# Fahien/rayca

Hardware: AMD Instinct MI355X
Metric: Mrays/sec (primary+shadow), 1920x1080 Sponza 1spp (higher is better)
Workload: dtype f32; 1 GPU; sponza-STAND-IN procedural atrium 271,568 tris, 1920x1080, primary + 1 shadow ray (Pathtracer max_depth=1, NEE, 1 point light), 1 spp; width=1920, height=1080, triangles=271568, bvh_nodes=135379, bvh_built_on=gpu (bvh_build.hip; same tree as the host builder), rays_per_frame=4146938, frames_in_flight=4, tiling=rows in bands of 8 dealt over 1 rank(s), frame_gather=none, launched_by=single process

## Files before the change

### rayca_amd/csrc/kernels.hip

```cpp
#include "no_pk.hpp"
RAYCA_NO_PK_BEGIN
#include <hip/hip_runtime.h>
#include "device_types.hpp"
RAYCA_NO_PK_END

namespace rayca {
namespace {

RAYCA_NO_PK_BEGIN
#include "trace_core.inc"

template <int MODE, bool GEN0, bool ORDERED, bool FUSED, bool FAST, bool SPH, bool WIDE, bool SPILL, bool STATS, bool HALF>
__global__ __launch_bounds__(kBlock, MODE == kModeFlat ? RAYCA_MIN_WAVES_FLAT : RAYCA_MIN_WAVES) void k_generation(DevScene sc, FrameParams fp, uint32_t* heads, const QueuedRay* in_rays,
                                                       const uint32_t* in_count, QueuedRay* out_rays, uint32_t* out_count,
                                                       PathBuffers pb, uint32_t depth, uint8_t* rgba8, float4* rgba32f,
                                                       TraceCounters* counters, TraceLaunch tl) {
  extern __shared__ uint32_t lds_stack[];
  NodeStack<SPILL> stack = make_stack<SPILL>(lds_stack, tl, rc_bid() * kBlock + rc_tid());
  float4* const ctx_slot = reinterpret_cast<float4*>(lds_stack + tl.lds_entries * kBlock) + rc_tid();
  constexpr bool PARK = RAYCA_PARK_CTX && MODE == kModePath;
  const uint32_t lane = __lane_id();
  const uint32_t home = xcc_id();
  WorkCursor wc{};
  const uint32_t total = GEN0 ? fp.tile_count : (*in_count + 63u) / 64u;
  LaneCounters cnt{};
  uint32_t n_shaded = 0, n_shadow = 0, n_bounce = 0;
  const bool collect_emissive = GEN0 ? true : (fp.direct_sampler == RAYCA_SAMPLER_NONE);
  const uint32_t nee_lights = (MODE == kModePath && fp.direct_sampler == RAYCA_SAMPLER_NEE) ? sc.light_count : 0u;

  for (;;) {
    const uint32_t batch = next_batch(heads, total, home, wc, tl.ticket);
    if (batch == RAYCA_NONE) break;
    bool live;
    uint32_t p = 0, key = 0;
    DRay ray;
    if (GEN0) {
      const uint32_t ty = batch / fp.tiles_x, tx = batch - ty * fp.tiles_x;
      const uint32_t x = tx * kTileW + (lane & (kTileW - 1u)), r = ty * kTileH + (lane >> RAYCA_TILE_W_LOG2);
      live = x < fp.width && r < fp.rows;
      const uint32_t y = ((r / fp.band) * fp.parts + fp.part) * fp.band + (r % fp.band);
      p = r * fp.width + x;
      if (live) {
        ray = camera_ray(fp, x, y);
        key = rng_root(fp.seed, y * fp.width + x, fp.sample);
      }
    } else {
      const uint32_t i = batch * 64u + lane;
      live = i < *in_count;
      if (live) {
        const QueuedRay q = in_rays[i];
        ray = make_ray(point3(q.ox, q.oy, q.oz), vec3(q.dx, q.dy, q.dz));
        p = q.pixel;
        key = q.key;
      }
    }
    const size_t slot = (size_t)depth * pb.npix + p;
    bool in_shadow = false;
    float t_stop = FLT_MAX;
    ShadeCtx cx;
    Color ns_x = black();
    Color direct = black();
    uint32_t li = 0, k = 0, dim = 0;
    const bool has_pixel = live;
    bool tail = false;

    while (live) {
      DHit hit;
      constexpr int kLeaveK = !ORDERED ? 0 : (MODE == kModeFlat ? RAYCA_LEAVE_K_CAMERA : (GEN0 ? RAYCA_LEAVE_K_PATH0 : RAYCA_LEAVE_K_BOUNCE));
      constexpr int kSlackForm = MODE == kModeFlat ? kSlackAlways : (GEN0 ? kSlackPerWave : kSlackNever);
      const bool found = trace<ORDERED, FAST, SPH, WIDE, SPILL, STATS, HALF, kLeaveK, kSlackForm>(sc, ray, t_stop, stack, hit, cnt);
      if (!in_shadow) {
        if (!found) {
          if (FUSED) direct = black() + black();
          else pb.state[slot] = kVertexNone;
          live = false;
        } else {
          n_shaded++;
          Color color;
          bool emissive;
          shade_hit<SPH>(sc, ray, hit, MODE == kModePath, color, emissive, cx);
          if (MODE == kModeFlat) {
            if (FUSED) direct = black() + color;
            else {
              pb.direct[slot] = as_f4(color);
              pb.state[slot] = kVertexEmissive;
            }
            live = false;
          } else if (collect_emissive && emissive) {
            pb.direct[slot] = as_f4(color);
            pb.state[slot] = kVertexEmissive;
            live = false;
          } else {
            in_shadow = true;
            if (PARK) {
              park_ctx(ctx_slot, cx);
              ctx_slot[6 * kBlock] = as_f4(black());
            }
          }
        }
      } else {
        bool lit;
        if (t_stop == FLT_MAX) {
          lit = false;
          if (found) {
            const uint32_t hm = sc.ext[hit.prim].material;
            lit = hm != RAYCA_NONE && hm < sc.material_count && sc.materials[hm].emissive != 0u;
          }
        } else {
          lit = !(found && hit.t < t_stop);
        }
        if (PARK) {
          const Color sum = as_color(ctx_slot[6 * kBlock]) + (lit ? as_color(ctx_slot[5 * kBlock]) : black());
          ctx_slot[6 * kBlock] = as_f4(sum);
        } else {
          direct = direct + (lit ? ns_x : black());
        }
        if (++k == fp.light_samples) {
          k = 0;
          ++li;
        }
      }
      if (live && in_shadow) {
        bool pending = false;
        while (li < nee_lights) {
          if (PARK) cx = unpark_ctx(ctx_slot);
          const NeeSample ns = nee_prepare(sc, fp, cx, li, k, key, dim, ray);
          const bool irrelevant = ORDERED && nee_irrelevant(ns);
          if (STATS) {
            const unsigned long long m = __ballot(irrelevant);
            if (m != 0ull && lane == (uint32_t)__ffsll((long long)m) - 1u) atomicAdd(&counters->nee_irrelevant, (unsigned long long)__popcll(m));
          }
          if (irrelevant && fp.nee_skip) {
            if (++k == fp.light_samples) {
              k = 0;
              ++li;
            }
            continue;
          }
          if (PARK) ctx_slot[5 * kBlock] = as_f4(ns.x);
          else ns_x = ns.x;
          t_stop = ns.t_stop;
          pending = true;
          break;
        }
        if (!pending) {
          tail = true;
          live = false;
        }
      }
    }
    if (FUSED) {
      if (has_pixel) finalize_pixel(fp, direct, p, rgba8, rgba32f);
    } else if (MODE == kModePath) {
      bool want_bounce = false;
      QueuedRay next{};
      if (tail) {
        const uint32_t limit = fp.direct_sampler != RAYCA_SAMPLER_NONE ? fp.max_depth - 1u : fp.max_depth;
        const bool hemi = fp.indirect_sampler == RAYCA_SAMPLER_HEMISPHERE;
        F4 sdir = vec3(0.0f, 0.0f, 0.0f);
        if (depth < limit) {
          const float e1 = rng_f32(key, dim++), e2 = rng_f32(key, dim++);
          const float theta = hemi ? rc_acosf(e1) : rc_acosf(sqrtf(e1));
          const float omega_a = 2.0f * kPi * e2;
          const float st = rc_sinf(theta);
          sdir = vec3(rc_cosf(omega_a) * st, rc_sinf(omega_a) * st, rc_cosf(theta));
        }
        if (PARK) {
          cx = unpark_ctx(ctx_slot);
          direct = as_color(ctx_slot[6 * kBlock]);
        }
        pb.direct[slot] = as_f4(direct);
        if (depth < limit) {
          const F4 w = cx.normal;
          const F4 a = close(w, vec3(0, 1, 0)) ? vec3(1, 0, 0) : vec3(0, 1, 0);
          const F4 u = normalized(cross(a, w));
          F4 v = cross(w, u);
          if (hemi) v = normalized(v);
          const F4 omega_i = (sdir.x * u + sdir.y * v) + sdir.z * w;
          const Color brdf = surf_brdf(cx, omega_i);
          Color factor;
          if (hemi) factor = ((2.0f * kPi) * brdf) * clampf(dot(cx.normal, omega_i), 0.0f, 1.0f);
          else factor = kPi * brdf;
          pb.brdf[slot] = as_f4(factor);
          pb.state[slot] = kVertexLit;
          if (depth + 1u < fp.max_depth) {
            want_bounce = true;
            next.ox = cx.next_origin.x; next.oy = cx.next_origin.y; next.oz = cx.next_origin.z;
            next.dx = omega_i.x; next.dy = omega_i.y; next.dz = omega_i.z;
            next.pixel = p;
            next.key = rng_child(key, 0u);
          }
        } else {
          pb.state[slot] = kVertexLitNoIndirect;
        }
      }
      n_shadow += (uint32_t)__popcll(__ballot(tail)) * nee_lights * fp.light_samples;
      n_bounce += (uint32_t)__popcll(__ballot(want_bounce));
      push_ray(want_bounce, next, out_rays, out_count);
    }
  }
  if (STATS) {
    unsigned long long b = cnt.boxes, t = cnt.tris, sh = n_shaded, sb = cnt.slot_boxes, stt = cnt.slot_tris;
    for (int off = 32; off > 0; off >>= 1) {
      b += __shfl_down(b, off);
      t += __shfl_down(t, off);
      sh += __shfl_down(sh, off);
      sb += __shfl_down(sb, off);
      stt += __shfl_down(stt, off);
    }
    if (lane == 0) {
      atomicAdd(&counters->boxes, b);
      atomicAdd(&counters->tris, t);
      atomicAdd(&counters->shaded, sh);
      atomicAdd(&counters->box_slots, sb);
      atomicAdd(&counters->tri_slots, stt);
    }
  }
  if (MODE == kModePath) {
    const unsigned long long s2 = n_shadow, b2 = n_bounce;
    if (lane == 0 && (s2 | b2)) {
      atomicAdd(&counters->shadow, s2);
      atomicAdd(&counters->bounce, b2);
    }
  }
}

__global__ __launch_bounds__(kBlock) void k_resolve(FrameParams fp, PathBuffers pb, uint32_t depths, float4* accum, uint8_t* rgba8, float4* rgba32f,
                                                    uint32_t* clear, uint32_t clear_words) {
  if (clear && rc_bid() == 0)
    for (uint32_t i = rc_tid(); i < clear_words; i += rc_bdim()) clear[i] = 0u;
  const uint32_t p = rc_bid() * rc_bdim() + rc_tid();
  if (p >= pb.npix) return;
  bool some = false;
  Color L = black();
  for (int g = (int)depths - 1; g >= 0; --g) {
    const size_t slot = (size_t)g * pb.npix + p;
    const uint32_t st = pb.state[slot];
    if (st == kVertexNone) {
      some = false;
    } else if (st == kVertexEmissive) {
      some = true;
      L = as_color(pb.direct[slot]);
    } else {
      const Color direct = as_color(pb.direct[slot]);
      Color indirect = black();
      if (st == kVertexLit) {
        Color li = black();
        if (some) {
          const Color factor = as_color(pb.brdf[slot]);
          const Color x = (factor * L) * 1.0f;
          li = li + x;
        }
        indirect = indirect + li / (float)fp.light_samples;
      }
      L = direct + indirect;
      some = true;
    }
  }
  const Color c = some ? L : black();
  const Color prev = fp.sample == 0 ? black() : as_color(accum[p]);
  const Color acc = prev + c;
  if (fp.sample + 1u == fp.spp) finalize_pixel(fp, acc, p, rgba8, rgba32f);
  else accum[p] = as_f4(acc);
}

template <bool ORDERED, bool FAST, bool SPH, bool WIDE, bool SPILL, bool STATS>
__global__ __launch_bounds__(kBlock, RAYCA_TRACE_MIN_WAVES) void k_trace_rays(DevScene sc, const float* rays, uint32_t count, float* t_out, uint32_t* prim_out, float* uv_out,
                                                       TraceCounters* counters, TraceLaunch tl) {
  extern __shared__ uint32_t lds_stack[];
  NodeStack<SPILL> stack = make_stack<SPILL>(lds_stack, tl, rc_bid() * kBlock + rc_tid());
  const uint32_t i = rc_bid() * rc_bdim() + rc_tid();
  LaneCounters cnt{};
  if (i < count) {
    const float* r = rays + 6ull * i;
    const DRay ray = make_ray(point3(r[0], r[1], r[2]), vec3(r[3], r[4], r[5]));
    DHit hit;
    const bool found = trace<ORDERED, FAST, SPH, WIDE, SPILL, STATS, false, 0, kSlackAlways>(sc, ray, FLT_MAX, stack, hit, cnt);
    t_out[i] = found ? hit.t : FLT_MAX;
    prim_out[i] = found ? hit.prim : RAYCA_NONE;
    uv_out[2 * i] = found ? hit.u : 0.0f;
    uv_out[2 * i + 1] = found ? hit.v : 0.0f;
  }
  if (STATS) {
    unsigned long long b = cnt.boxes, t = cnt.tris;
    for (int off = 32; off > 0; off >>= 1) {
      b += __shfl_down(b, off);
      t += __shfl_down(t, off);
    }
    if (__lane_id() == 0) {
      atomicAdd(&counters->boxes, b);
      atomicAdd(&counters->tris, t);
    }
  }
}

template <bool ORDERED, bool FAST, bool SPH, bool WIDE, bool SPILL, bool STATS, bool OCCLUDED>
__global__ __launch_bounds__(kBlock, RAYCA_TRACE_MIN_WAVES) void k_query_rays(DevScene sc, QueryIo q, TraceCounters* counters, TraceLaunch tl) {
  extern __shared__ uint32_t lds_stack[];
  NodeStack<SPILL> stack = make_stack<SPILL>(lds_stack, tl, rc_bid() * kBlock + rc_tid());
  const uint32_t i = rc_bid() * rc_bdim() + rc_tid();
  LaneCounters cnt{};
  if (i < q.count) {
    bool dead;
    const float bound = query_bound(q, i, dead);
    DHit hit;
    hit.t = INFINITY;
    hit.prim = RAYCA_NONE;
    hit.u = hit.v = 0.0f;
    if (!dead) {
      const float* r = q.rays + 6ull * i;
      const DRay ray = make_ray(point3(r[0], r[1], r[2]), vec3(r[3], r[4], r[5]));
      const float t_stop = !OCCLUDED ? FLT_MAX : (bound < FLT_MAX ? bound : __uint_as_float(0x7F7FFFFEu));
      trace<ORDERED, FAST, SPH, WIDE, SPILL, STATS, false, 0, kSlackAlways>(sc, ray, t_stop, stack, hit, cnt);
    }
    query_store<OCCLUDED>(q, i, hit, query_found(hit, bound));
  }
  if (STATS) {
    unsigned long long b = cnt.boxes, t = cnt.tris;
    for (int off = 32; off > 0; off >>= 1) {
      b += __shfl_down(b, off);
      t += __shfl_down(t, off);
    }
    if (__lane_id() == 0) {
      atomicAdd(&counters->boxes, b);
      atomicAdd(&counters->tris, t);
    }
  }
}

#include "general.inc"
#include "wavefront.inc"
#include "surface.inc"
RAYCA_NO_PK_END
#include "denoise.inc"
#include "denoise_variance.inc"
#include "temporal.inc"
#include "upsample.inc"

}
}

#include "api.inc"
```

### rayca_amd/csrc/trace_core.inc

```
constexpr int kBlock = 256;
#ifndef RAYCA_TRACE_MIN_WAVES
#define RAYCA_TRACE_MIN_WAVES 1
#endif
#ifndef RAYCA_MIN_WAVES_FLAT
#define RAYCA_MIN_WAVES_FLAT 5
#endif
#ifndef RAYCA_MIN_WAVES
#define RAYCA_MIN_WAVES 4
#endif

__device__ __forceinline__ uint32_t rc_tid() { return __builtin_amdgcn_workitem_id_x(); }
__device__ __forceinline__ uint32_t rc_bid() { return __builtin_amdgcn_workgroup_id_x(); }
__device__ __forceinline__ uint32_t rc_bdim() { return __builtin_amdgcn_workgroup_size_x(); }
__device__ __forceinline__ uint32_t rc_gdim() { return __builtin_amdgcn_grid_size_x() / __builtin_amdgcn_workgroup_size_x(); }

struct DRay {
  F4 o, d, rd;
};
struct DHit {
  float t;
  uint32_t prim;
  float u, v;
};

__device__ __forceinline__ DRay make_ray(F4 origin, F4 dir) {
  DRay r;
  r.rd = reciprocal(dir);
  origin.w = 1.0f;
  r.o = origin;
  r.d = dir;
  return r;
}

__device__ __forceinline__ bool slab(float ax, float ay, float az, float bx, float by, float bz, const DRay& r, float& tmin_out) {
  const float t1x = __fmaf_rn(ax - r.o.x, r.rd.x, 0.0f), t2x = __fmaf_rn(bx - r.o.x, r.rd.x, 0.0f);
  const float t1y = __fmaf_rn(ay - r.o.y, r.rd.y, 0.0f), t2y = __fmaf_rn(by - r.o.y, r.rd.y, 0.0f);
  const float t1z = __fmaf_rn(az - r.o.z, r.rd.z, 0.0f), t2z = __fmaf_rn(bz - r.o.z, r.rd.z, 0.0f);
  const float tmax = fminf(fminf(fmaxf(t1x, t2x), fmaxf(t1y, t2y)), fminf(fmaxf(t1z, t2z), FLT_MAX));
  const float tmin = fmaxf(fmaxf(fminf(t1x, t2x), fminf(t1y, t2y)), fmaxf(fminf(t1z, t2z), -FLT_MAX));
  tmin_out = tmin;
  return tmax >= tmin && tmax > 0.0f;
}

#ifndef RAYCA_RAY_SLACK
#define RAYCA_RAY_SLACK 1
#endif
struct FastRay {
  float mx, my, mz, cx, cy, cz;
#if RAYCA_RAY_SLACK
  float slack;
  bool fixed;
#endif
};
__device__ __forceinline__ bool fix_axis(float& m, float& c, float o, float centre, float inv_scale) {
  if (fabsf(c) <= FLT_MAX && fabsf(m) <= FLT_MAX) return false;
  const float d = centre - o;
  if (!(fabsf(d) <= FLT_MAX)) {
    m = 0.0f;
    c = -FLT_MAX;
    return true;
  }
  const float big = copysignf(fminf(1.2676506002282294e30f, 1.329227995784916e36f / fabsf(d)), m);
  m = big * inv_scale;
  c = d * big;
  return true;
}
__device__ __forceinline__ FastRay make_fast(const DevScene& sc, const DRay& r, bool half) {
  FastRay f;
  if (half) {
    f.mx = r.rd.x * sc.half_inv_scale; f.my = r.rd.y * sc.half_inv_scale; f.mz = r.rd.z * sc.half_inv_scale;
    f.cx = (sc.half_center[0] - r.o.x) * r.rd.x; f.cy = (sc.half_center[1] - r.o.y) * r.rd.y; f.cz = (sc.half_center[2] - r.o.z) * r.rd.z;
  } else {
    f.mx = r.rd.x; f.my = r.rd.y; f.mz = r.rd.z;
    f.cx = -(r.o.x * r.rd.x); f.cy = -(r.o.y * r.rd.y); f.cz = -(r.o.z * r.rd.z);
  }
#if RAYCA_RAY_SLACK
  f.fixed = fix_axis(f.mx, f.cx, r.o.x, half ? sc.half_center[0] : 0.0f, half ? sc.half_inv_scale : 1.0f);
  f.fixed |= fix_axis(f.my, f.cy, r.o.y, half ? sc.half_center[1] : 0.0f, half ? sc.half_inv_scale : 1.0f);
  f.fixed |= fix_axis(f.mz, f.cz, r.o.z, half ? sc.half_center[2] : 0.0f, half ? sc.half_inv_scale : 1.0f);
  f.slack = fmaxf(fmaxf(fabsf(f.cx), fabsf(f.cy)), fabsf(f.cz)) * 4.76837158203125e-07f;
#endif
  return f;
}
__device__ __forceinline__ bool ray_needs_slack(const DevScene& sc, const DRay& r, const FastRay& f) {
#if RAYCA_RAY_SLACK
  const float radius = sc.cull_abs * 4096.0f;
  return !(fabsf(r.o.x) <= radius && fabsf(r.o.y) <= radius && fabsf(r.o.z) <= radius) || f.fixed;
#else
  return false;
#endif
}
template <bool SLACK>
__device__ __forceinline__ bool slab_verdict(float tmin, float tmax, const FastRay& f) {
#if RAYCA_RAY_SLACK
  if (SLACK) {
    const float tp = tmax + f.slack;
    return tp >= tmin && tp > 0.0f;
  }
#endif
  return tmax >= tmin && tmax > 0.0f;
}
template <bool SLACK>
__device__ __forceinline__ float cull_limit(const DevScene& sc, const FastRay& f, float b) {
#if RAYCA_RAY_SLACK
  if (SLACK) return b + fabsf(b) * 9.765625e-4f + sc.cull_abs + f.slack;
#endif
  return b + fabsf(b) * 9.765625e-4f + sc.cull_abs;
}
typedef _Float16 rc_h2 __attribute__((ext_vector_type(2)));
__device__ __forceinline__ float lo16(uint32_t w) { return (float)__builtin_bit_cast(rc_h2, w).x; }
__device__ __forceinline__ float hi16(uint32_t w) { return (float)__builtin_bit_cast(rc_h2, w).y; }
template <bool SLACK>
__device__ __forceinline__ bool slab_fast(float ax, float ay, float az, float bx, float by, float bz, const FastRay& f, float& tmin_out) {
  const float t1x = __fmaf_rn(ax, f.mx, f.cx), t2x = __fmaf_rn(bx, f.mx, f.cx);
  const float t1y = __fmaf_rn(ay, f.my, f.cy), t2y = __fmaf_rn(by, f.my, f.cy);
  const float t1z = __fmaf_rn(az, f.mz, f.cz), t2z = __fmaf_rn(bz, f.mz, f.cz);
  const float tmax = fminf(fminf(fmaxf(t1x, t2x), fmaxf(t1y, t2y)), fmaxf(t1z, t2z));
  const float tmin = fmaxf(fmaxf(fminf(t1x, t2x), fminf(t1y, t2y)), fminf(t1z, t2z));
  tmin_out = tmin;
  return slab_verdict<SLACK>(tmin, tmax, f);
}
#ifndef RAYCA_NODE_CH
#define RAYCA_NODE_CH 1
#endif
#ifndef RAYCA_NODE_CH48
#define RAYCA_NODE_CH48 1
#endif
constexpr uint32_t kChNodeQuads = RAYCA_NODE_CH48 ? 3u : 4u;
constexpr uint32_t kChRefScale = RAYCA_NODE_CH48 ? 48u : 1u;
#ifndef RAYCA_WF_PRIMARY_WIDE
#define RAYCA_WF_PRIMARY_WIDE 0
#endif
#ifndef RAYCA_WF_PRIMARY_HALF
#define RAYCA_WF_PRIMARY_HALF 1
#endif
#ifndef RAYCA_WF_BOUNCE_WIDE
#define RAYCA_WF_BOUNCE_WIDE 1
#endif
#ifndef RAYCA_WF_BOUNCE_HALF
#define RAYCA_WF_BOUNCE_HALF 1
#endif
#ifndef RAYCA_WF_SHADOW_WIDE
#define RAYCA_WF_SHADOW_WIDE 1
#endif
#ifndef RAYCA_WF_SHADOW_HALF
#define RAYCA_WF_SHADOW_HALF 1
#endif
template <bool SLACK>
__device__ __forceinline__ bool slab_ch(float cx, float cy, float cz, float hx, float hy, float hz, const FastRay& f, float& tmin_out) {
  const float tx = __fmaf_rn(cx, f.mx, f.cx), ty = __fmaf_rn(cy, f.my, f.cy), tz = __fmaf_rn(cz, f.mz, f.cz);
  const float ex = fabsf(f.mx), ey = fabsf(f.my), ez = fabsf(f.mz);
  const float nx = __fmaf_rn(-hx, ex, tx), ny = __fmaf_rn(-hy, ey, ty), nz = __fmaf_rn(-hz, ez, tz);
  const float fx = __fmaf_rn(hx, ex, tx), fy = __fmaf_rn(hy, ey, ty), fz = __fmaf_rn(hz, ez, tz);
  const float tmax = fminf(fminf(fx, fy), fz);
  const float tmin = fmaxf(fmaxf(nx, ny), nz);
  tmin_out = tmin;
  return slab_verdict<SLACK>(tmin, tmax, f);
}
template <bool SLACK>
__device__ __forceinline__ bool slab_half(float ax, float ay, float az, float bx, float by, float bz, const FastRay& f, float& tmin_out) {
  return slab_fast<SLACK>(ax, ay, az, bx, by, bz, f, tmin_out);
}

__device__ __forceinline__ bool tri_test(F4 v0, F4 v1, F4 v2, const DRay& r, float& t_out, float& u_out, float& v_out) {
  const F4 v0v1 = v1 - v0;
  const F4 v0v2 = v2 - v0;
  const F4 n = cross(v0v1, v0v2);
  if (dot(r.d, n) > 0.0f) return false;
  const float denom = dot(n, n);
  const float ndd = dot(n, r.d);
  if (fabsf(ndd) < FLT_EPSILON) return false;
  const float d = -dot(n, v0);
  const float t = -(dot(n, to_vec(r.o)) + d) / ndd;
  if (t < 0.0f) return false;
  const F4 p = r.o + r.d * t;
  F4 c = cross(v1 - v0, to_vec(p - v0));
  if (dot(n, c) < 0.0f) return false;
  c = cross(v2 - v1, to_vec(p - v1));
  const float u = dot(n, c);
  if (u < 0.0f) return false;
  c = cross(v0 - v2, to_vec(p - v2));
  const float v = dot(n, c);
  if (v < 0.0f) return false;
  t_out = t;
  u_out = u / denom;
  v_out = v / denom;
  return true;
}

__device__ __forceinline__ DRay sphere_local_ray(const DevSphere& sp, const DRay& r) {
  F4 o = r.o + (-f4(sp.translation[0], sp.translation[1], sp.translation[2], 0.0f));
  F4 d = r.d;
  const F4 iq = f4(sp.inv_rotation[0], sp.inv_rotation[1], sp.inv_rotation[2], sp.inv_rotation[3]);
  d = rotate(d, iq);
  o = point_rotate(o, iq);
  o.w = 1.0f;
  const F4 is = f4(sp.inv_scale[0], sp.inv_scale[1], sp.inv_scale[2], sp.inv_scale[3]);
  d = d * is;
  o = point_scale(o, is);
  DRay l;
  l.o = o;
  l.d = d;
  l.rd = reciprocal(d);
  return l;
}
__device__ __forceinline__ bool sphere_test(const DevSphere& sp, const DRay& r, float& t_out) {
  const DRay l = sphere_local_ray(sp, r);
  const F4 center = f4(sp.center[0], sp.center[1], sp.center[2], sp.center[3]);
  const float a = dot(l.d, l.d);
  const F4 c_to_r = as_vec(l.o - center);
  const float b = dot(c_to_r, l.d);
  const float c = dot(c_to_r, c_to_r) - sp.radius2;
  const float det = b * b - a * c;
  if (det < 0.0f) return false;
  const float det_sqrt = sqrtf(det);
  const float t0 = (-b + det_sqrt) / a;
  const float t1 = (-b - det_sqrt) / a;
  if (t0 < 0.0f && t1 < 0.0f) return false;
  float t;
  if (t0 >= 0.0f && t1 >= 0.0f) t = fminf(t0, t1);
  else if (t0 >= 0.0f) t = t0;
  else t = t1;
  t_out = t;
  return true;
}

struct TriRecord {
  F4 v0, v1, v2;
  uint32_t rank, leaf;
};
constexpr uint32_t kTriQuads = 3, kTriFloats = 12;
__device__ __forceinline__ TriRecord load_tri(const DevScene& sc, uint32_t i) {
  const float4* p = sc.tris + (size_t)kTriQuads * i;
  const float4 q0 = p[0], q1 = p[1], q2 = p[2];
  TriRecord t;
  t.v0 = vec3(q0.x, q0.y, q0.z);
  t.v1 = vec3(q0.w, q1.x, q1.y);
  t.v2 = vec3(q1.z, q1.w, q2.x);
  t.rank = __float_as_uint(q2.y);
  t.leaf = __float_as_uint(q2.z);
  return t;
}

__device__ __forceinline__ bool tie_before(const DevScene& sc, uint32_t rank_a, uint32_t b) {
  if (b == RAYCA_NONE) return true;
  const uint32_t rank_b = __float_as_uint(reinterpret_cast<const float*>(sc.tris)[(size_t)kTriFloats * b + 9u]);
  return rank_a < rank_b;
}

__device__ __forceinline__ bool reference_candidate(const DevScene& sc, const TriRecord& t, const DRay& r) {
  if (!sc.ref_leaf_of) return true;
  const float4* b = sc.ref_leaf_boxes + 2ull * t.leaf;
  const float4 lo = b[0], hi = b[1];
  float tmin;
  return slab(lo.x, lo.y, lo.z, hi.x, hi.y, hi.z, r, tmin);
}

struct LaneCounters {
  uint32_t boxes, tris;
  unsigned long long slot_boxes, slot_tris;
  __device__ __forceinline__ bool books() const { return __lane_id() == (uint32_t)__ffsll((long long)__ballot(1)) - 1u; }
};

constexpr uint32_t kTerminated = 0x7FFFFFFFu;

template <bool SPILL>
struct NodeStack {
  uint32_t* lds;
  uint32_t* ovf;
  uint32_t gthread;
  uint32_t lds_entries, ovf_stride, sp;
  uint32_t top;
  __device__ __forceinline__ void clear() { sp = 0; top = kTerminated; }
#ifndef RAYCA_STACK_AS
#define RAYCA_STACK_AS 1
#endif
  typedef __attribute__((address_space(3))) uint32_t LdsWord;
  typedef __attribute__((address_space(1))) uint32_t GlobalWord;
  __device__ __forceinline__ void put(uint32_t i, uint32_t v) {
#if RAYCA_STACK_AS
    if (!SPILL || i < lds_entries) ((LdsWord*)lds)[i * kBlock] = v;
    else ((GlobalWord*)ovf)[(size_t)(i - lds_entries) * ovf_stride + gthread] = v;
#else
    if (!SPILL || i < lds_entries) lds[i * kBlock] = v;
    else ovf[(size_t)(i - lds_entries) * ovf_stride + gthread] = v;
#endif
  }
  __device__ __forceinline__ uint32_t get(uint32_t i) const {
#if RAYCA_STACK_AS
    uint32_t v;
    if (!SPILL || i < lds_entries) v = ((const LdsWord*)lds)[i * kBlock];
    else v = ((const GlobalWord*)ovf)[(size_t)(i - lds_entries) * ovf_stride + gthread];
    return v;
#else
    return (!SPILL || i < lds_entries) ? lds[i * kBlock] : ovf[(size_t)(i - lds_entries) * ovf_stride + gthread];
#endif
  }
  __device__ __forceinline__ void push(uint32_t v) {
    if (top != kTerminated) put(sp++, top);
    top = v;
  }
  __device__ __forceinline__ uint32_t pop() {
    const uint32_t r = top;
    if (sp == 0) top = kTerminated;
    else top = get(--sp);
    return r;
  }
};
template <bool SPILL>
__device__ __forceinline__ NodeStack<SPILL> make_stack(uint32_t* lds_base, const TraceLaunch& tl, uint32_t global_thread) {
  NodeStack<SPILL> st;
  st.lds = lds_base + rc_tid();
  st.ovf = tl.ovf;
  st.gthread = global_thread;
  st.lds_entries = tl.lds_entries;
  st.ovf_stride = tl.ovf_stride;
  st.clear();
  return st;
}

template <bool ORDERED, bool SPH, bool STATS, bool SLACK = true>
__device__ __forceinline__ void test_leaf(const DevScene& sc, const DRay& r, const FastRay& fr, uint32_t ref, float t_stop, DHit& hit, float& limit,
                                          LaneCounters& cnt) {
  const uint32_t first = ref & kLeafFirstMask;
  const uint32_t count = ((ref >> 25) & 63u) + 1u;
  for (uint32_t i = first; i < first + count; ++i) {
    const TriRecord tr = load_tri(sc, i);
    if (STATS) {
      cnt.tris++;
      if (cnt.books()) cnt.slot_tris += 64ull;
    }
    float t, u, v;
    bool got;
    if (SPH && tr.v0.x != tr.v0.x) {
      u = v = 0.0f;
      got = sphere_test(sc.spheres[__float_as_uint(tr.v0.y)], r, t);
    } else {
      got = tri_test(tr.v0, tr.v1, tr.v2, r, t, u, v);
    }
    if (got) {
      if ((t < hit.t || (t == hit.t && tie_before(sc, tr.rank, hit.prim))) && reference_candidate(sc, tr, r)) {
        hit.t = t;
        hit.prim = i;
        hit.u = u;
        hit.v = v;
        if (ORDERED) {
          limit = cull_limit<SLACK>(sc, fr, fminf(t, t_stop));
        }
      }
    }
  }
}

template <bool ORDERED, bool FAST, bool WIDE, bool SPILL, bool STATS, bool HALF, bool SLACK = true>
__device__ __forceinline__ uint32_t node_step(const DevScene& sc, const DRay& r, const FastRay& fr, float limit, uint32_t cur, NodeStack<SPILL>& st,
                                              LaneCounters& cnt) {
  if (STATS && cnt.books()) cnt.slot_boxes += WIDE ? 256ull : 128ull;
  if (WIDE) {
    float key[4];
    uint32_t ref[4];
    if (FAST && HALF) {
      const uint4* np = sc.nodes4_h + 4ull * cur;
      const uint4 q0 = np[0], q1 = np[1], q2 = np[2], q3 = np[3];
      if (STATS) cnt.boxes += 4;
      ref[0] = q3.x; ref[1] = q3.y; ref[2] = q3.z; ref[3] = q3.w;
      const float ax[4] = {lo16(q0.x), hi16(q0.x), lo16(q0.y), hi16(q0.y)}, ay[4] = {lo16(q0.z), hi16(q0.z), lo16(q0.w), hi16(q0.w)};
      const float az[4] = {lo16(q1.x), hi16(q1.x), lo16(q1.y), hi16(q1.y)}, bx[4] = {lo16(q1.z), hi16(q1.z), lo16(q1.w), hi16(q1.w)};
      const float by[4] = {lo16(q2.x), hi16(q2.x), lo16(q2.y), hi16(q2.y)}, bz[4] = {lo16(q2.z), hi16(q2.z), lo16(q2.w), hi16(q2.w)};
#pragma unroll
      for (int c = 0; c < 4; ++c) {
        float tc;
        bool h = slab_half<SLACK>(ax[c], ay[c], az[c], bx[c], by[c], bz[c], fr, tc);
        if (ORDERED) h = h && tc <= limit;
        key[c] = h ? (ORDERED ? tc : (float)c) : INFINITY;
      }
    } else {
    const float4* np = sc.nodes4 + 8ull * cur;
    const float4 lx = np[0], ly = np[1], lz = np[2], hx = np[3], hy = np[4], hz = np[5], cr = np[6];
    if (STATS) cnt.boxes += 4;
    ref[0] = __float_as_uint(cr.x); ref[1] = __float_as_uint(cr.y); ref[2] = __float_as_uint(cr.z); ref[3] = __float_as_uint(cr.w);
    const float ax[4] = {lx.x, lx.y, lx.z, lx.w}, ay[4] = {ly.x, ly.y, ly.z, ly.w}, az[4] = {lz.x, lz.y, lz.z, lz.w};
    const float bx[4] = {hx.x, hx.y, hx.z, hx.w}, by[4] = {hy.x, hy.y, hy.z, hy.w}, bz[4] = {hz.x, hz.y, hz.z, hz.w};
#pragma unroll
    for (int c = 0; c < 4; ++c) {
      float tc;
      bool h = FAST ? slab_fast<SLACK>(ax[c], ay[c], az[c], bx[c], by[c], bz[c], fr, tc) : slab(ax[c], ay[c], az[c], bx[c], by[c], bz[c], r, tc);
      if (ORDERED) h = h && tc <= limit;
      key[c] = h ? (ORDERED ? tc : (float)c) : INFINITY;
    }
    }
#define RC_CE(i, j)                                  \
  {                                                  \
const bool sw = key[i] > key[j];                 \
const float ka = sw ? key[j] : key[i];           \
const float kb = sw ? key[i] : key[j];           \
const uint32_t ra = sw ? ref[j] : ref[i];        \
const uint32_t rb = sw ? ref[i] : ref[j];        \
key[i] = ka; key[j] = kb; ref[i] = ra; ref[j] = rb; \
  }
    RC_CE(0, 1) RC_CE(2, 3) RC_CE(0, 2) RC_CE(1, 3) RC_CE(1, 2)
#undef RC_CE
    if (key[3] < INFINITY) st.push(ref[3]);
    if (key[2] < INFINITY) st.push(ref[2]);
    if (key[1] < INFINITY) st.push(ref[1]);
    cur = key[0] < INFINITY ? ref[0] : st.pop();
  } else {
    float tl, tr;
    bool hl, hr;
    uint32_t lref, rref;
    if (FAST && HALF) {
      const uint4* nh = sc.nodes_h + 2ull * cur;
      const uint4 a = nh[0], b = nh[1];
      hl = slab_half<SLACK>(lo16(a.x), hi16(a.x), lo16(a.y), hi16(a.y), lo16(a.z), hi16(a.z), fr, tl);
      hr = slab_half<SLACK>(lo16(a.w), hi16(a.w), lo16(b.x), hi16(b.x), lo16(b.y), hi16(b.y), fr, tr);
      lref = b.z;
      rref = b.w;
    } else {
      if (FAST && RAYCA_NODE_CH && RAYCA_NODE_CH48) {
        const float4* np = reinterpret_cast<const float4*>(reinterpret_cast<const char*>(sc.nodes_ch) + cur);
        const float4 q0 = np[0], q1 = np[1], q2 = np[2];
        hl = slab_ch<SLACK>(q0.x, q0.y, q0.z, q0.w, q1.x, q1.y, fr, tl);
        hr = slab_ch<SLACK>(q1.z, q1.w, q2.x, q2.y, q2.z, q2.w, fr, tr);
        lref = __builtin_amdgcn_perm(__float_as_uint(q1.x), __float_as_uint(q0.w), 0x05040100u);
        rref = __builtin_amdgcn_perm(__float_as_uint(q2.z), __float_as_uint(q2.y), 0x05040100u);
      } else {
        const float4* np = (FAST && RAYCA_NODE_CH ? sc.nodes_ch : sc.nodes) + 4ull * cur;
        const float4 q0 = np[0], q1 = np[1], q2 = np[2], q3 = np[3];
        if (FAST && RAYCA_NODE_CH) {
          hl = slab_ch<SLACK>(q0.x, q0.y, q0.z, q0.w, q1.x, q1.y, fr, tl);
          hr = slab_ch<SLACK>(q1.z, q1.w, q2.x, q2.y, q2.z, q2.w, fr, tr);
        } else if (FAST) {
          hl = slab_fast<SLACK>(q0.x, q0.y, q0.z, q0.w, q1.x, q1.y, fr, tl);
          hr = slab_fast<SLACK>(q1.z, q1.w, q2.x, q2.y, q2.z, q2.w, fr, tr);
        } else {
          hl = slab(q0.x, q0.y, q0.z, q0.w, q1.x, q1.y, r, tl);
          hr = slab(q1.z, q1.w, q2.x, q2.y, q2.z, q2.w, r, tr);
        }
        lref = __float_as_uint(q3.x);
        rref = __float_as_uint(q3.y);
      }
    }
    if (STATS) cnt.boxes += 2;
    if (ORDERED) {
      hl = hl && tl <= limit;
      hr = hr && tr <= limit;
    }
    if (hl && hr) {
      const bool left_first = !ORDERED || tl <= tr;
      st.push(left_first ? rref : lref);
      cur = left_first ? lref : rref;
    } else if (hl) {
      cur = lref;
    } else if (hr) {
      cur = rref;
    } else {
      cur = st.pop();
    }
  }
  return cur;
}

#ifndef RAYCA_LEAVE_K_CAMERA
#define RAYCA_LEAVE_K_CAMERA 0
#endif
#ifndef RAYCA_LEAVE_K_PATH0
#define RAYCA_LEAVE_K_PATH0 0
#endif
#ifndef RAYCA_LEAVE_K_BOUNCE
#define RAYCA_LEAVE_K_BOUNCE 8
#endif
template <bool ORDERED, bool FAST, bool SPH, bool WIDE, bool SPILL, bool STATS, bool HALF, int LEAVE_K, bool SLACK>
__device__ __forceinline__ bool trace_search(const DevScene& sc, const DRay& r, const FastRay& fr, float t_stop, NodeStack<SPILL>& st, DHit& hit, LaneCounters& cnt) {
  hit.t = INFINITY;
  hit.prim = RAYCA_NONE;
  hit.u = hit.v = 0.0f;
  float tmin;
  if (STATS) cnt.boxes++;
  uint32_t cur = WIDE ? sc.root_ref4 : (FAST && !HALF && RAYCA_NODE_CH ? sc.root_ref_ch : sc.root_ref);
  if (!slab(sc.root_min[0], sc.root_min[1], sc.root_min[2], sc.root_max[0], sc.root_max[1], sc.root_max[2], r, tmin)) cur = kTerminated;
  st.clear();
  const bool any_hit = ORDERED && t_stop < FLT_MAX;
  float limit = INFINITY;
  if (any_hit) limit = cull_limit<SLACK>(sc, fr, t_stop);
  if constexpr (LEAVE_K > 0) {
  for (;;) {
    for (;;) {
      const bool searching = !(cur & kLeafFlag) && cur != kTerminated;
      const uint32_t n = (uint32_t)__popcll(__ballot(searching));
      if (n == 0u) break;
      if (n < (uint32_t)LEAVE_K && __ballot((cur & kLeafFlag) != 0u) != 0ull) break;
      if (searching) cur = node_step<ORDERED, FAST, WIDE, SPILL, STATS, HALF, SLACK>(sc, r, fr, limit, cur, st, cnt);
    }
    if ((cur & kLeafFlag) && cur != kTerminated) {
      test_leaf<ORDERED, SPH, STATS, SLACK>(sc, r, fr, cur, t_stop, hit, limit, cnt);
      cur = (any_hit && hit.t < t_stop) ? kTerminated : st.pop();
    }
    if (__ballot(cur != kTerminated) == 0ull) break;
  }
  } else {
  while (cur != kTerminated) {
    while (!(cur & kLeafFlag) && cur != kTerminated) {
      cur = node_step<ORDERED, FAST, WIDE, SPILL, STATS, HALF, SLACK>(sc, r, fr, limit, cur, st, cnt);
    }
    if (cur != kTerminated) {
      test_leaf<ORDERED, SPH, STATS, SLACK>(sc, r, fr, cur, t_stop, hit, limit, cnt);
      if (any_hit && hit.t < t_stop) break;
      cur = st.pop();
    }
  }
  }
  return hit.prim != RAYCA_NONE;
}

constexpr int kSlackPerWave = 0, kSlackAlways = 1, kSlackNever = 2;
template <bool ORDERED, bool FAST, bool SPH, bool WIDE, bool SPILL, bool STATS, bool HALF = false, int LEAVE_K = 0, int SLACK_FORM = kSlackPerWave>
__device__ __forceinline__ bool trace(const DevScene& sc, const DRay& r, float t_stop, NodeStack<SPILL>& st, DHit& hit, LaneCounters& cnt) {
  const FastRay fr = make_fast(sc, r, HALF);
  if constexpr (!FAST || !RAYCA_RAY_SLACK || SLACK_FORM == kSlackNever) {
    return trace_search<ORDERED, FAST, SPH, WIDE, SPILL, STATS, HALF, LEAVE_K, false>(sc, r, fr, t_stop, st, hit, cnt);
  } else if constexpr (SLACK_FORM == kSlackAlways) {
    return trace_search<ORDERED, FAST, SPH, WIDE, SPILL, STATS, HALF, LEAVE_K, true>(sc, r, fr, t_stop, st, hit, cnt);
  } else {
    if (__ballot(ray_needs_slack(sc, r, fr)) != 0ull)
      return trace_search<ORDERED, FAST, SPH, WIDE, SPILL, STATS, HALF, LEAVE_K, true>(sc, r, fr, t_stop, st, hit, cnt);
    return trace_search<ORDERED, FAST, SPH, WIDE, SPILL, STATS, HALF, LEAVE_K, false>(sc, r, fr, t_stop, st, hit, cnt);
  }
}

__device__ __forceinline__ float query_bound(const QueryIo& q, uint32_t i, bool& dead) {
  const float tm = q.tmax ? q.tmax[i] : q.tmax_all;
  dead = !(tm > 0.0f);
  return tm < FLT_MAX ? tm : FLT_MAX;
}
__device__ __forceinline__ bool query_found(const DHit& hit, float bound) { return hit.prim != RAYCA_NONE && (bound == FLT_MAX || hit.t < bound); }
template <bool OCCLUDED>
__device__ __forceinline__ void query_store(const QueryIo& q, uint32_t i, const DHit& hit, bool found) {
  if (OCCLUDED) {
    q.occluded_out[i] = found ? 1 : 0;
  } else {
    if (q.t_out) q.t_out[i] = found ? hit.t : FLT_MAX;
    if (q.prim_out) q.prim_out[i] = found ? hit.prim : RAYCA_NONE;
    if (q.uv_out) {
      q.uv_out[2ull * i] = found ? hit.u : 0.0f;
      q.uv_out[2ull * i + 1ull] = found ? hit.v : 0.0f;
    }
  }
}

__device__ __forceinline__ Color load_color(const float* c) { return Color{c[0], c[1], c[2], c[3]}; }
__device__ __forceinline__ F4 load_vec3(const float* c) { return vec3(c[0], c[1], c[2]); }

__device__ __forceinline__ uint32_t f32_as_u32_sat(float v) {
  if (!(v == v) || v <= 0.0f) return 0u;
  if (v >= 4294967296.0f) return 0xFFFFFFFFu;
  return (uint32_t)v;
}
__device__ Color sample_texture(const DevScene& sc, uint32_t tex, F2 uv) {
  const DevTexture t = sc.textures[tex];
  const float fx = (uv.x - floorf(uv.x) + 1.0f) * (float)t.width;
  const float fy = (uv.y - floorf(uv.y) + 1.0f) * (float)t.height;
  const uint32_t x = f32_as_u32_sat(fx) % t.width, y = f32_as_u32_sat(fy) % t.height;
  const size_t idx = (size_t)y * t.width + x;
  const uint8_t* base = sc.image_bytes + t.byte_offset;
  if (t.color_type == RAYCA_COLOR_RGBA32F) {
    const float* f = reinterpret_cast<const float*>(base) + idx * 4;
    return Color{f[0] / 255.0f, f[1] / 255.0f, f[2] / 255.0f, f[3] / 255.0f};
  }
  if (t.color_type == RAYCA_COLOR_RGBA8) {
    const uint8_t* p = base + idx * 4;
    return Color{(float)p[0] / 255.0f, (float)p[1] / 255.0f, (float)p[2] / 255.0f, (float)p[3] / 255.0f};
  }
  const uint8_t* p = base + idx * 3;
  return Color{(float)p[0] / 255.0f, (float)p[1] / 255.0f, (float)p[2] / 255.0f, 255.0f / 255.0f};
}

__device__ __forceinline__ bool tex_valid(const DevScene& sc, uint32_t t) { return t != RAYCA_NONE && t < sc.texture_count; }

__device__ __forceinline__ Color pbr_color(const DevScene& sc, const DevMaterial& m, F2 uv) {
  const Color c = load_color(m.color);
  if (tex_valid(sc, m.albedo_texture)) return c * sample_texture(sc, m.albedo_texture, uv);
  return c;
}
__device__ __forceinline__ void pbr_metallic_roughness(const DevScene& sc, const DevMaterial& m, F2 uv, float& metallic, float& roughness) {
  if (tex_valid(sc, m.metallic_roughness_texture)) {
    const Color c = sample_texture(sc, m.metallic_roughness_texture, uv);
    metallic = c.b;
    roughness = c.r;
  } else {
    metallic = m.metallic_factor;
    roughness = m.roughness_factor;
  }
}
__device__ __forceinline__ DevMaterial default_material() {
  DevMaterial m{};
  m.color[0] = m.color[1] = m.color[2] = m.color[3] = 1.0f;
  m.ambient[3] = m.emission[3] = m.diffuse[3] = m.specular[3] = 1.0f;
  m.kind = RAYCA_MATERIAL_PBR;
  m.albedo_texture = m.normal_texture = m.metallic_roughness_texture = RAYCA_NONE;
  m.metallic_factor = 0.0f;
  m.roughness_factor = 1.0f;
  return m;
}

__device__ __forceinline__ F4 interp3(const float (*a)[3], float bu, float bv) {
  const float w2 = 1.0f - bu - bv;
  return (load_vec3(a[2]) * w2 + load_vec3(a[0]) * bu) + load_vec3(a[1]) * bv;
}

struct ShadeCtx {
  F4 point, normal, view, next_origin;
  Color kd, ks;
  float roughness, shininess;
  uint32_t kind;
};

#ifndef RAYCA_PARK_CTX
#define RAYCA_PARK_CTX 1
#endif
constexpr uint32_t kCtxQuads = 7;
__device__ __forceinline__ void park_ctx(float4* slot, const ShadeCtx& c) {
  slot[0 * kBlock] = make_float4(c.point.x, c.point.y, c.point.z, c.roughness);
  slot[1 * kBlock] = make_float4(c.normal.x, c.normal.y, c.normal.z, c.shininess);
  slot[2 * kBlock] = make_float4(c.view.x, c.view.y, c.view.z, __uint_as_float(c.kind));
  slot[3 * kBlock] = make_float4(c.kd.r, c.kd.g, c.kd.b, c.kd.a);
  slot[4 * kBlock] = make_float4(c.ks.r, c.ks.g, c.ks.b, c.ks.a);
}
__device__ __forceinline__ ShadeCtx unpark_ctx(const float4* slot) {
  const float4 q0 = slot[0 * kBlock], q1 = slot[1 * kBlock], q2 = slot[2 * kBlock], q3 = slot[3 * kBlock], q4 = slot[4 * kBlock];
  ShadeCtx c;
  c.point = f4(q0.x, q0.y, q0.z, 1.0f);
  c.normal = vec3(q1.x, q1.y, q1.z);
  c.view = vec3(q2.x, q2.y, q2.z);
  c.next_origin = c.point + c.normal * kRayBias;
  c.kd = Color{q3.x, q3.y, q3.z, q3.w};
  c.ks = Color{q4.x, q4.y, q4.z, q4.w};
  c.roughness = q0.w;
  c.shininess = q1.w;
  c.kind = __float_as_uint(q2.w);
  return c;
}

template <bool SPH>
__device__ __forceinline__ void shade_hit(const DevScene& sc, const DRay& ray, const DHit& hit, bool full, Color& color, bool& emissive,
                                          ShadeCtx& cx) {
  const PrimExt& e = sc.ext[hit.prim];
  const float bu = hit.u, bv = hit.v;
  const float w2 = 1.0f - bu - bv;
  const bool is_sphere = SPH && e.kind == RAYCA_GEOMETRY_SPHERE;
  const Color geom_color = is_sphere ? white() : (load_color(e.color[2]) * w2 + load_color(e.color[0]) * bu) + load_color(e.color[1]) * bv;
  const F2 uv = is_sphere ? F2{0.0f, 0.0f}
                          : F2{(e.uv[2][0] * w2 + e.uv[0][0] * bu) + e.uv[1][0] * bv, (e.uv[2][1] * w2 + e.uv[0][1] * bu) + e.uv[1][1] * bv};
  const DevMaterial m = (e.material != RAYCA_NONE && e.material < sc.material_count) ? sc.materials[e.material] : default_material();
  Color mc;
  if (m.kind == RAYCA_MATERIAL_PBR) mc = pbr_color(sc, m, uv);
  else if (m.kind == RAYCA_MATERIAL_PHONG) mc = load_color(m.ambient) + load_color(m.emission);
  else mc = load_color(m.diffuse);
  color = geom_color * mc;
  emissive = m.emissive != 0u;
  if (!full) return;
  F4 normal;
  F4 point = ray.o + ray.d * hit.t;
  F4 hit_dir = ray.d;
  if (is_sphere) {
    const DevSphere& sp = sc.spheres[e.node];
    const DRay l = sphere_local_ray(sp, ray);
    hit_dir = l.d;
    const F4 model_point = l.o + l.d * hit.t;
    const Trs wt{f4(sp.translation[0], sp.translation[1], sp.translation[2], 0.0f), f4(sp.rotation[0], sp.rotation[1], sp.rotation[2], sp.rotation[3]),
                 f4(sp.scale[0], sp.scale[1], sp.scale[2], 0.0f)};
    point = trs_apply_point(wt, model_point);
    const F4 hp = mat4_apply_point(reinterpret_cast<const float(*)[4]>(sp.inv_mat4), point);
    const F4 mn = normalized(as_vec(hp - f4(sp.center[0], sp.center[1], sp.center[2], sp.center[3])));
    const float* nm = sp.normal_mat;
    float out[3] = {0.0f, 0.0f, 0.0f};
    const float in[3] = {mn.x, mn.y, mn.z};
    for (int i = 0; i < 3; ++i)
      for (int j = 0; j < 3; ++j) out[i] += nm[4 * i + j] * in[j];
    normal = normalized(vec3(out[0], out[1], out[2]));
  } else {
    normal = normalized(interp3(e.normal, bu, bv));
  }
  if (!is_sphere && m.kind == RAYCA_MATERIAL_PBR && tex_valid(sc, m.normal_texture)) {
    const F4 tangent = normalized(interp3(e.tangent, bu, bv));
    const F4 bitangent = normalized(interp3(e.bitangent, bu, bv));
    F4 sn = premultiplied(sample_texture(sc, m.normal_texture, uv));
    sn = sn * 2.0f - f4(1.0f, 1.0f, 1.0f, 1.0f);
    normal = normalized(mat3_apply(mat3_tbn(tangent, bitangent, normal), sn));
  }
  cx.normal = normal;
  cx.point = point;
  cx.view = -hit_dir;
  cx.next_origin = cx.point + normal * kRayBias;
  cx.kind = m.kind;
  cx.shininess = m.shininess;
  if (m.kind == RAYCA_MATERIAL_PBR) {
    float me, ro;
    pbr_metallic_roughness(sc, m, uv, me, ro);
    const Color base = pbr_color(sc, m, uv);
    cx.kd = geom_color * base;
    cx.ks = me * base;
    cx.roughness = ro;
  } else {
    cx.kd = geom_color * load_color(m.diffuse);
    cx.ks = load_color(m.specular);
    cx.roughness = m.kind == RAYCA_MATERIAL_PHONG ? clampf(sqrtf(2.0f / (m.shininess + 2.0f)), 0.0f, 1.0f) : m.roughness_factor;
  }
}

#ifndef RAYCA_GGX_CLOSED_FORM
#define RAYCA_GGX_CLOSED_FORM 1
#endif
__device__ __forceinline__ float ggx_d(float a, F4 h, F4 n) {
  const float a2 = a * a;
  const float cos_theta = clampf(dot(h, n), 0.0f, 1.0f);
#if RAYCA_GGX_CLOSED_FORM
  const float q = a2 * (cos_theta * cos_theta) + (1.0f - cos_theta) * (1.0f + cos_theta);
  const float denominator = q * q;
  if (denominator == 0.0f || cos_theta == 0.0f) return 0.0f;
#else
  const float theta = acosf(cos_theta);
  const float denominator = powf(cos_theta, 4.0f) * powf(a2 + powf(tanf(theta), 2.0f), 2.0f);
  if (denominator == 0.0f) return 0.0f;
#endif
  return a2 * kFrac1Pi / denominator;
}
__device__ __forceinline__ float ggx_g1(float a, F4 omega, F4 n) {
  const float cos_theta = dot(omega, n);
  if (cos_theta <= 0.0f) return 0.0f;
#if RAYCA_GGX_CLOSED_FORM
  const float tan2 = cos_theta > 1.0f ? NAN : ((1.0f - cos_theta) * (1.0f + cos_theta)) / (cos_theta * cos_theta);
  return 2.0f / (1.0f + sqrtf(1.0f + a * a * tan2));
#else
  const float theta = acosf(cos_theta);
  return 2.0f / (1.0f + sqrtf(1.0f + a * a * powf(tanf(theta), 2.0f)));
#endif
}
__device__ __forceinline__ Color ggx_f(Color ks, F4 omega_i, F4 h) {
  const float oh = fabsf(dot(omega_i, h));
#if RAYCA_GGX_CLOSED_FORM
  const float x = 1.0f - oh, x2 = x * x;
  return ks + (white() - ks) * ((x2 * x2) * x);
#else
  return ks + (white() - ks) * powf(1.0f - oh, 5.0f);
#endif
}
__device__ __forceinline__ Color surf_brdf(const ShadeCtx& s, F4 omega_i) {
  if (s.kind == RAYCA_MATERIAL_PHONG) {
    const Color lambertian = s.kd * kFrac1Pi;
    const float sh = s.shininess;
    const F4 refl = normalized(reflect(-s.view, s.normal));
    const Color specular = (((s.ks * (sh + 2.0f)) * powf(dot(refl, omega_i), sh)) * kFrac1Pi) / 2.0f;
    return lambertian + specular;
  }
  Color bsdf = black();
  const F4 omega_o = s.view;
  const F4 n = s.normal;
  const float oin = clampf(dot(omega_i, n), 0.0f, 1.0f);
  const float oon = clampf(dot(omega_o, n), 0.0f, 1.0f);
  if (!(oin == 0.0f || oon == 0.0f)) {
    const float a = s.roughness;
    const F4 h = normalized(omega_i + omega_o);
    const Color f = ggx_f(s.ks, omega_i, h);
    const float g = ggx_g1(a, omega_i, n) * ggx_g1(a, omega_o, n);
    const float d = ggx_d(a, h, n);
    const float denominator = 4.0f * oin * oon;
    bsdf = ((f * g) * d) / denominator;
  }
  return s.kd * kFrac1Pi + bsdf;
}

__device__ __forceinline__ uint32_t xcc_id() {
  uint32_t v;
  asm volatile("s_getreg_b32 %0, hwreg(HW_REG_XCC_ID)" : "=s"(v));
  return v & 7u;
}
constexpr uint32_t kHeadStride = 64;
struct WorkCursor {
  uint32_t exhausted;
  uint32_t next, end;
};
__device__ __forceinline__ uint32_t next_batch(uint32_t* heads, uint32_t total, uint32_t home, WorkCursor& wc, uint32_t ticket) {
  if (wc.next < wc.end) return wc.next++;
  ticket = max(ticket, 1u);
  while (wc.exhausted < 8u) {
    const uint32_t part = (home + wc.exhausted) & 7u;
    const uint32_t lo = (uint32_t)(((uint64_t)part * total) >> 3), hi = (uint32_t)(((uint64_t)(part + 1u) * total) >> 3);
    uint32_t idx = 0;
    if (__lane_id() == 0) idx = atomicAdd(&heads[part * kHeadStride], ticket);
    idx = __builtin_amdgcn_readfirstlane(idx);
    if (idx < hi - lo) {
      wc.next = lo + idx + 1u;
      wc.end = min(lo + idx + ticket, hi);
      return lo + idx;
    }
    wc.exhausted++;
  }
  return RAYCA_NONE;
}

struct PathBuffers {
  float4* direct;
  float4* brdf;
  uint32_t* state;
  uint32_t npix;
};

__device__ __forceinline__ float4 as_f4(Color c) { return make_float4(c.r, c.g, c.b, c.a); }
__device__ __forceinline__ Color as_color(float4 c) { return Color{c.x, c.y, c.z, c.w}; }

__device__ __forceinline__ void finalize_pixel(const FrameParams& fp, Color acc, uint32_t p, uint8_t* rgba8, float4* rgba32f) {
  Color c = acc / (float)fp.spp;
  if (fp.inv_gamma != 1.0f) {
    c.r = powf(c.r, fp.inv_gamma);
    c.g = powf(c.g, fp.inv_gamma);
    c.b = powf(c.b, fp.inv_gamma);
  }
  if (rgba32f) rgba32f[p] = as_f4(c);
  if (rgba8) {
    const uint32_t packed = (uint32_t)quantize(c.r) | ((uint32_t)quantize(c.g) << 8) | ((uint32_t)quantize(c.b) << 16) | ((uint32_t)quantize(c.a) << 24);
    reinterpret_cast<uint32_t*>(rgba8)[p] = packed;
  }
}

__device__ __forceinline__ DRay camera_ray(const FrameParams& fp, uint32_t x, uint32_t y) {
  const float xx = (2.0f * ((((float)x + fp.sub_step_x) + fp.sub_offset) * fp.inv_width) - 1.0f) * fp.angle * fp.aspect;
  const float yy = (1.0f - 2.0f * ((((float)y + fp.sub_step_y) + fp.sub_offset) * fp.inv_height)) * fp.angle;
  F4 dir = normalized(vec3(xx, yy, -1.0f));
  F4 origin = point3(0.0f, 0.0f, 0.0f);
  dir = dir * fp.camera.scale;
  origin = point_scale(origin, fp.camera.scale);
  dir = rotate(dir, fp.camera.rotation);
  origin = point_rotate(origin, fp.camera.rotation);
  origin.w = 1.0f;
  origin = origin + fp.camera.translation;
  DRay r;
  r.o = origin;
  r.d = dir;
  r.rd = reciprocal(dir);
  return r;
}

__device__ __forceinline__ void push_ray(bool has, const QueuedRay& qr, QueuedRay* out, uint32_t* out_count) {
  const unsigned long long mask = __ballot(has);
  if (mask == 0ull) return;
  const uint32_t lane = __lane_id();
  const uint32_t leader = (uint32_t)__ffsll((long long)mask) - 1u;
  uint32_t base = 0;
  if (lane == leader) base = atomicAdd(out_count, (uint32_t)__popcll(mask));
  base = __shfl(base, (int)leader);
  if (has) out[base + (uint32_t)__popcll(mask & ((1ull << lane) - 1ull))] = qr;
}

constexpr int kModeFlat = 0, kModePath = 1, kModeGeneral = 2;

struct NeeSample {
  Color x;
  float t_stop;
  uint32_t quad;
};
__device__ __forceinline__ NeeSample nee_prepare(const DevScene& sc, const FrameParams& fp, const ShadeCtx& s, uint32_t li, uint32_t k,
                                                 uint32_t key, uint32_t& dim, DRay& shadow_ray) {
  const DevLight L = sc.lights[li];
  NeeSample ns;
  const F4 x_point = s.point;
  if (L.kind == RAYCA_LIGHT_POINT) {
    const F4 x1 = f4(L.position[0], L.position[1], L.position[2], L.position[3]);
    const F4 x_to_x1 = as_vec(x1 - x_point);
    const float dist = length(x_to_x1);
    const F4 omega = normalized(x_to_x1);
    shadow_ray = make_ray(s.next_origin, omega);
    const F4 dvec = to_vec(x_point) - to_vec(x1);
    const float r2 = norm2(dvec);
    const float rr = sqrtf(r2);
    const float fallof = hsum(f4(L.attenuation[0], L.attenuation[1], L.attenuation[2], 0.0f) * f4(1.0f, rr, r2, 0.0f));
    const Color le = (L.intensity * load_color(L.color)) / fallof;
    const Color brdf = surf_brdf(s, omega);
    const float r_squared = norm2(x_to_x1);
    const float d_omega = 1.0f / r_squared;
    const float n_dot_omega = clampf(dot(s.normal, omega), 0.0f, 1.0f);
    ns.x = ((le * brdf) * n_dot_omega) * d_omega;
    ns.t_stop = dist;
    ns.quad = 0u;
  } else {
    const F4 ab = f4(L.ab[0], L.ab[1], L.ab[2], 0.0f), ac = f4(L.ac[0], L.ac[1], L.ac[2], 0.0f);
    const float sc_f = (float)fp.strate_count;
    const float u1 = rng_f32(key, dim++) / sc_f;
    const float u2 = rng_f32(key, dim++) / sc_f;
    const F4 a = f4(L.position[0], L.position[1], L.position[2], L.position[3]);
    F4 x1 = (a + u1 * ab) + u2 * ac;
    if (fp.light_stratify) {
      const float i1 = (float)(k % fp.strate_count), i2 = (float)(k / fp.strate_count);
      x1 = x1 + ((ab / sc_f) * i1 + (ac / sc_f) * i2);
    }
    const F4 x_to_x1 = as_vec(x1 - x_point);
    const F4 omega = normalized(x_to_x1);
    shadow_ray = make_ray(s.next_origin, omega);
    const Color le = L.intensity * load_color(L.color);
    const Color brdf = surf_brdf(s, omega);
    const float r_squared = norm2(x_to_x1);
    const float d_omega = dot(f4(L.normal[0], L.normal[1], L.normal[2], 0.0f), omega) / r_squared;
    const float n_dot_omega = clampf(dot(s.normal, omega), 0.0f, 1.0f);
    ns.x = (((le * L.area) * brdf) * n_dot_omega) * d_omega;
    ns.t_stop = FLT_MAX;
    ns.quad = 1u;
  }
  return ns;
}

__device__ __forceinline__ bool nee_irrelevant(const NeeSample& ns) {
  return ns.x.r == 0.0f && ns.x.g == 0.0f && ns.x.b == 0.0f && fabsf(ns.x.a) < INFINITY;
}
constexpr uint32_t kShadowQuad = 1u, kShadowSkip = 2u;

struct WfBuffers {
  float4* hits;
  float4* sh_ray;
  float4* sh_x;
  uint32_t nls;
};

__device__ __forceinline__ bool tile_item_pixel(const FrameParams& fp, uint32_t item, uint32_t& x, uint32_t& r) {
  const uint32_t batch = item >> 6, j = item & 63u;
  if (batch >= fp.tile_count) return false;
  const uint32_t ty = batch / fp.tiles_x, tx = batch - ty * fp.tiles_x;
  x = tx * kTileW + (j & (kTileW - 1u));
  r = ty * kTileH + (j >> RAYCA_TILE_W_LOG2);
  return x < fp.width && r < fp.rows;
}
```

Baseline: 13700 Mrays/s.

## Prefetch next BVH node before stack bookkeeping in compressed-node traversal

Adds a specialised ordered traversal loop for the 48-byte compressed node layout. It issues the load of the next node before doing the stack push/pop bookkeeping, so node fetch latency overlaps with LDS or global stack traffic. The stack update becomes a branchless transfer with a wave-uniform check for spill. The parked context initialisation is also changed to build the zero float4 from an opaque register. This adds code complexity, and correctness depends on the new stack bookkeeping matching the old semantics.

```diff
diff --git a/rayca_amd/csrc/kernels.hip b/rayca_amd/csrc/kernels.hip
--- a/rayca_amd/csrc/kernels.hip
+++ b/rayca_amd/csrc/kernels.hip
@@ -94,7 +94,9 @@
             in_shadow = true;
             if (PARK) {
               park_ctx(ctx_slot, cx);
-              ctx_slot[6 * kBlock] = as_f4(black());
+              float zero = 0.0f;
+              asm volatile("" : "+v"(zero));
+              ctx_slot[6 * kBlock] = make_float4(zero, zero, zero, 1.0f);
             }
           }
         }
diff --git a/rayca_amd/csrc/trace_core.inc b/rayca_amd/csrc/trace_core.inc
--- a/rayca_amd/csrc/trace_core.inc
+++ b/rayca_amd/csrc/trace_core.inc
@@ -304,6 +304,37 @@
     const uint32_t r = top;
     if (sp == 0) top = kTerminated;
     else top = get(--sp);
+    return r;
+  }
+  __device__ __forceinline__ void transfer(bool wr, bool rd, uint32_t at, bool keep, uint32_t v, uint32_t& out) {
+    if (SPILL && __ballot(sp >= lds_entries) != 0ull) {
+      const bool deep = at >= lds_entries;
+      GlobalWord* const g = (GlobalWord*)ovf + ((size_t)(at - lds_entries) * ovf_stride + gthread);
+      if (wr && deep) *g = top;
+      if (rd && deep) {
+        v = *g;
+        asm volatile("" : "+v"(v));
+        keep = false;
+      }
+      wr = wr && !deep;
+      rd = rd && !deep;
+    }
+    if (wr) ((LdsWord*)lds)[at * kBlock] = top;
+    asm volatile("" : "+v"(top), "+v"(out));
+    top = keep ? top : v;
+    if (rd) top = ((const LdsWord*)lds)[at * kBlock];
+  }
+  __device__ __forceinline__ void book(bool both, bool none, uint32_t far, uint32_t& cur) {
+    const bool wr = both && top != kTerminated, rd = none && sp != 0u;
+    const uint32_t at = rd ? sp - 1u : sp;
+    transfer(wr, rd, at, !(both || none), both ? far : kTerminated, cur);
+    sp = wr ? sp + 1u : at;
+  }
+  __device__ __forceinline__ uint32_t pop_late(bool take) {
+    uint32_t r = take ? top : kTerminated;
+    const bool rd = take && sp != 0u;
+    sp -= rd ? 1u : 0u;
+    transfer(false, rd, sp, !take, kTerminated, r);
     return r;
   }
 };
@@ -497,6 +528,38 @@
     }
     if (__ballot(cur != kTerminated) == 0ull) break;
   }
+  } else if constexpr (ORDERED && FAST && !WIDE && !HALF && RAYCA_NODE_CH && RAYCA_NODE_CH48) {
+  while (cur != kTerminated) {
+    if (!(cur & kLeafFlag)) {
+      const float4* np = reinterpret_cast<const float4*>(reinterpret_cast<const char*>(sc.nodes_ch) + cur);
+      float4 q0 = np[0], q1 = np[1], q2 = np[2];
+      bool more;
+      do {
+        if (STATS && cnt.books()) cnt.slot_boxes += 128ull;
+        float tl, tr;
+        bool hl = slab_ch<SLACK>(q0.x, q0.y, q0.z, q0.w, q1.x, q1.y, fr, tl);
+        bool hr = slab_ch<SLACK>(q1.z, q1.w, q2.x, q2.y, q2.z, q2.w, fr, tr);
+        const uint32_t lref = __builtin_amdgcn_perm(__float_as_uint(q1.x), __float_as_uint(q0.w), 0x05040100u);
+        const uint32_t rref = __builtin_amdgcn_perm(__float_as_uint(q2.z), __float_as_uint(q2.y), 0x05040100u);
+        if (STATS) cnt.boxes += 2;
+        hl = hl && tl <= limit;
+        hr = hr && tr <= limit;
+        const bool left_first = tl <= tr;
+        const bool both = hl && hr, none = !(hl || hr);
+        cur = none ? st.top : ((hl && (left_first || !hr)) ? lref : rref);
+        more = !(cur & kLeafFlag) && cur != kTerminated;
+        if (more) {
+          const float4* nn = reinterpret_cast<const float4*>(reinterpret_cast<const char*>(sc.nodes_ch) + cur);
+          q0 = nn[0]; q1 = nn[1]; q2 = nn[2];
+        }
+        st.book(both, none, left_first ? rref : lref, cur);
+      } while (more);
+    }
+    if (cur != kTerminated) {
+      test_leaf<ORDERED, SPH, STATS, SLACK>(sc, r, fr, cur, t_stop, hit, limit, cnt);
+      cur = st.pop_late(!(any_hit && hit.t < t_stop));
+    }
+  }
   } else {
   while (cur != kTerminated) {
     while (!(cur & kLeafFlag) && cur != kTerminated) {
```

Result: faster. 14040 Mrays/s (median of 6 runs) (+2.5%).
